# constantingoeldel/alphabeta-rs

Measured on AMD Instinct MI355X. Metric: ABneutral model fits/sec (pedigree x bootstraps x windows), higher is better.
Workload: dtype f64; 1 GPU; C3: synthetic 100-edge/8-generation pedigree (N=105 rows, T=8, K=47 distinct triples), 10 starts + 10000 bootstraps per GPU (bootstraps of one window sharded over the GPUs); rows=105, windows_per_gpu=1, starts=10, bootstraps=10000, plan_device_bytes=9663014, reduction_tree=0x10040, parallelism=bootstraps sharded over 1 GPU(s), one RCCL all-gather of the bootstrap tables

## Files before the change

### alphabeta_rs_amd/csrc/abn_fit_refill.hpp

```cpp
#pragma once
#include "abn_common.hpp"
#include "abn_fit_kernel.hpp"

namespace abn {

constexpr int ST_IDLE = 13;

#ifndef ABN_REFILL_MIN_WAVES
#define ABN_REFILL_MIN_WAVES 3
#endif
template <int G, int RMAX>
__global__ __launch_bounds__(kWave, ABN_REFILL_MIN_WAVES) void abn_fit_refill_kernel(const FitArgs a) {
  static_assert(RMAX > 0, "resident mode only");
  constexpr int NG = kWave / G;
  constexpr int RR = RMAX;
  extern __shared__ __align__(16) double lds[];

  const int lane = threadIdx.x;
  const int g = lane / G;
  const int gl = lane - g * G;
  const int dim = gl & 3;
  const unsigned total = (unsigned)((long long)a.W * a.C);
  const int N = a.N, K = a.K, TP = a.TP;

  double* pw = lds + (size_t)g * a.chain_stride;
  double* dtab = pw + kPw * TP;
  double* wconst = dtab + ((K + 1) & ~1);
  double* dobs = wconst + 4;
  uint32_t* tri_s = reinterpret_cast<uint32_t*>(dobs + ((N + 1) & ~1));

  unsigned* const pht = a.quantum > 0 ? a.park_ht + (blockIdx.x & (kParkShards - 1)) * kParkHeaderInts : nullptr;
  int* const pk = a.quantum > 0 ? a.parked + (size_t)(blockIdx.x & (kParkShards - 1)) * a.park_cap : nullptr;
  const bool canon = a.tree == kTreeCanon;
  uint32_t tidp[(RR + 1) / 2];
  for (int t = gl; t < K; t += G) tri_s[t] = a.tri[t];
#pragma unroll
  for (int q = 0; q < (RR + 1) / 2; ++q) tidp[q] = 0u;
#pragma unroll
  for (int q = 0; q < RR; ++q) {
    const int i = gl + G * q;
    if (i < N) tidp[q / 2] |= (uint32_t)a.tid[i] << (16 * (q & 1));
  }

  unsigned chain = blockIdx.x * NG + g;
  double vx[5], c[5];
  int st = ST_IDLE;
  int iter = 0, evals = 0;
  double xc = 0.0, x0 = 0.0, xr = 0.0, bx = __builtin_nan("");
  double fr = 0.0, best_cost = __builtin_inf();
  bool have_best = false;
  int fin_status = 2;
  int q_start = 0;
  bool fresh_done = false;
  bool wave_fd = false;
  bool tail_mode = false;
  bool tail_park = false;
  unsigned wstep = 0;
#pragma unroll
  for (int k = 0; k < 5; ++k) {
    vx[k] = 0.0;
    c[k] = 0.0;
  }

  auto setup_chain = [&]() {
    const int w = (int)(chain / (unsigned)a.C);
    const int j = (int)(chain - (unsigned)w * (unsigned)a.C);
    const int wi = w * a.wstride;
    const size_t wN = (size_t)w * (size_t)N;
    if (gl == 0) {
      const double p_uu0 = a.p_uu[wi];
      wconst[0] = p_uu0;
      wconst[1] = 1.0 - p_uu0;
      wconst[2] = a.eqp[wi];
      wconst[3] = a.eqp_w[wi] * (double)N;
    }
    const uint32_t* idx_row = (a.dmode == 1) ? a.idx + (size_t)chain * (size_t)N : nullptr;
    const size_t dN = (a.dmode == 2) ? (size_t)chain * (size_t)N : wN;
#pragma unroll
    for (int q = 0; q < RR; ++q) {
      const int i = gl + G * q;
      if (i < N)
        dobs[i] = (a.dmode == 1) ? a.pred[wN + i] + a.resid[wN + idx_row[i]] : a.D[dN + i];
    }
    if (a.smode == 0) {
      const double* s0 = a.simplex0 + (size_t)chain * 20;
#pragma unroll
      for (int k = 0; k < 5; ++k) vx[k] = s0[4 * k + dim];
    } else {
      const uint32_t k0 = (uint32_t)a.seed, k1 = (uint32_t)(a.seed >> 32);
      const uint32_t wg = a.wid ? a.wid[w] : a.window_offset + (uint32_t)w, bg = a.boot_offset + (uint32_t)j;
      vx[0] = a.model[4 * w + dim];
#pragma unroll
      for (int v = 1; v < 5; ++v) {
        uint32_t r[4];
        philox4x32_10((uint32_t)(v - 1) * 2u + (uint32_t)(dim >> 1), bg, wg, kTagJitter, k0, k1, r);
        const uint32_t r0 = r[0], r1 = r[1], r2 = r[2], r3 = r[3];
        const bool odd = (dim & 1) != 0;
        vx[v] = vary_one(vx[0], odd ? r2 : r0, odd ? r3 : r1);
      }
    }
    iter = 0;
    evals = 0;
    bx = __builtin_nan("");
    best_cost = __builtin_inf();
    have_best = false;
    fin_status = 2;
    fr = 0.0;
    q_start = a.quantum > 0 ? -(int)((chain * 2654435761u >> 16) % (unsigned)a.quantum) : 0;
    st = ST_INIT0;
  };
  auto resume_chain = [&]() {
    const int w = (int)(chain / (unsigned)a.C);
    const int wi = w * a.wstride;
    const size_t wN = (size_t)w * (size_t)N;
    if (gl == 0) {
      const double p_uu0 = a.p_uu[wi];
      wconst[0] = p_uu0;
      wconst[1] = 1.0 - p_uu0;
      wconst[2] = a.eqp[wi];
      wconst[3] = a.eqp_w[wi] * (double)N;
    }
    const uint32_t* idx_row = (a.dmode == 1) ? a.idx + (size_t)chain * (size_t)N : nullptr;
    const size_t dN = (a.dmode == 2) ? (size_t)chain * (size_t)N : wN;
#pragma unroll
    for (int q = 0; q < RR; ++q) {
      const int i = gl + G * q;
      if (i < N)
        dobs[i] = (a.dmode == 1) ? a.pred[wN + i] + a.resid[wN + idx_row[i]] : a.D[dN + i];
    }
    double* sp = a.state + (size_t)chain * 32;
    auto ld = [&](int i) { return __hip_atomic_load(sp + i, __ATOMIC_RELAXED, __HIP_MEMORY_SCOPE_AGENT); };
#pragma unroll
    for (int k = 0; k < 5; ++k) {
      vx[k] = ld(4 * k + dim);
      c[k] = ld(20 + k);
    }
    bx = ld(25 + dim);
    best_cost = ld(29);
    const long long ie = __double_as_longlong(ld(30));
    iter = (int)(ie & 0xffffffffll);
    evals = (int)(ie >> 32);
    have_best = __double_as_longlong(ld(31)) != 0;
    fin_status = 2;
    fr = 0.0;
    double acc = vx[0];
    acc = acc + vx[1];
    acc = acc + vx[2];
    acc = acc + vx[3];
    x0 = acc * (1.0 / 4.0);
    xr = x0 + (x0 - vx[4]) * 1.0;
    xc = xr;
    q_start = evals;
    st = ST_REFLECT;
  };
  if (chain < total) setup_chain();
  __syncthreads();

  auto eval = [&](double xd) -> double {
    const double al = dpp_mov<kDppQuadBcast0>(xd), be = dpp_mov<kDppQuadBcast1>(xd);
    const double wt = dpp_mov<kDppQuadBcast2>(xd), ic = dpp_mov<kDppQuadBcast3>(xd);
    const double p_mm = wconst[1];
    const double sv0 = wconst[0], sv1 = wt * p_mm, sv2 = (1.0 - wt) * p_mm;
    const double puu = p_uu_est(al, be);
    const double dq = puu - wconst[2];
    const double pen = wconst[3] * (dq * dq);
    uint32_t tr = tri_s[gl < K ? gl : 0];
    if constexpr (kMatrixFma && G == kWave) build_power_table_mx<G>(al, be, a.T, lds, a.chain_stride, dtab, lane);
    else build_power_table<G>(genmatrix(al, be), a.T, TP, pw, gl);
    __syncthreads();
#pragma unroll 1
    for (int t = gl; t < K; t += G) {
      const uint32_t trn = tri_s[t + G < K ? t + G : 0];
      dtab[t] = triple_dt(tr, pw, TP, sv0, sv1, sv2);
      tr = trn;
    }
    __syncthreads();
    double acc = 0.0;
    constexpr int RC = RR < 8 ? RR : 8;
    constexpr int NA = kWave / G;
    double av[NA];
#pragma unroll
    for (int j = 0; j < NA; ++j) av[j] = 0.0;
#pragma unroll
    for (int q0 = 0; q0 < RR; q0 += RC) {
      double dv[RC], tv[RC], x[RC];
#pragma unroll
      for (int q = 0; q < RC; ++q) {
        const int i = gl + G * (q0 + q);
        dv[q] = dobs[i < N ? i : N - 1];
        tv[q] = dtab[(tidp[(q0 + q) / 2] >> (16 * ((q0 + q) & 1))) & 0xffffu];
      }
#pragma unroll
      for (int q = 0; q < RC; ++q) {
        const double r = dv[q] - ic - tv[q];
        const double term = r * r + pen;
        x[q] = ((gl + G * (q0 + q)) < N) ? term : 0.0;
      }
      if (canon) {
#pragma unroll
        for (int q = 0; q < RC; ++q) av[(q0 + q) % NA] = av[(q0 + q) % NA] + x[q];
      } else {
#pragma unroll
        for (int q = 0; q < RC; ++q) acc = acc + x[q];
      }
    }
    acc = canon ? tree64_finish<G>(av) : group_sum_dpp<G>(acc);
    __syncthreads();
    return acc;
  };

  auto begin_iteration = [&](bool count_iter) {
    const double c_best = c[0];
    if (c_best < best_cost || (__builtin_isinf(c_best) && __builtin_isinf(best_cost) &&
                               (__builtin_signbit(c_best) == __builtin_signbit(best_cost)))) {
      bx = vx[0];
      best_cost = c_best;
      have_best = true;
    }
    if (count_iter) ++iter;
    bool converged = false;
    if (!((c[4] - c[0]) > a.gap_tol)) {
      double sum = 0.0;
#pragma unroll
      for (int k = 0; k < 5; ++k) sum = sum + c[k];
      const double c0 = sum / 5.0;
      double ss = 0.0;
#pragma unroll
      for (int k = 0; k < 5; ++k) ss = ss + (c[k] - c0) * (c[k] - c0);
      const double sd = __builtin_sqrt(1.0 / (5.0 - 1.0) * ss);
      converged = sd < a.sd_tol;
    }
    int status = -1;
    if (converged) status = 0;
    else if (iter >= a.max_iters) status = 1;
    else if (best_cost <= -__builtin_inf()) status = 3;
    bool suspend = false;
    if (a.quantum > 0 && status < 0 && evals - q_start >= a.quantum) {
      int verdict = 0;
      if (gl == 0) {
        const unsigned fq = __hip_atomic_load(a.queue, __ATOMIC_RELAXED, __HIP_MEMORY_SCOPE_AGENT);
        const int av = __hip_atomic_load(reinterpret_cast<int*>(pht) + kParkAvail, __ATOMIC_RELAXED,
                                         __HIP_MEMORY_SCOPE_AGENT);
        const unsigned tl = __hip_atomic_load(pht + kParkTail, __ATOMIC_RELAXED, __HIP_MEMORY_SCOPE_AGENT);
        verdict = ((gridDim.x * NG + fq < total || av > 0) && tl + gridDim.x * NG / kParkShards + NG < a.park_cap) ? 1 : 0;
      }
      suspend = __builtin_amdgcn_ds_bpermute(4 * (g * G), verdict) != 0;
      q_start = evals;
    }
    tail_park = false;
    if (tail_mode && status < 0 && !suspend) {
      suspend = true;
      tail_park = true;
    }
    const bool done = status >= 0 || suspend;
    fin_status = (status >= 0) ? (have_best ? status : 2) : (suspend ? kFitSuspended : fin_status);
    double acc = vx[0];
    acc = acc + vx[1];
    acc = acc + vx[2];
    acc = acc + vx[3];
    x0 = acc * (1.0 / 4.0);
    xr = x0 + (x0 - vx[4]) * 1.0;
    xc = xr;
    st = done ? ST_DONE : ST_REFLECT;
  };

#ifdef ABN_MEASUREMENT_KNOBS
  int prio_cur = 0;
#endif
  while (__ballot(st != ST_IDLE) != 0ull) {
#ifdef ABN_MEASUREMENT_KNOBS
    if (a.prio_mode != 0) {
      const int e = st != ST_IDLE ? evals : 0;
      int m = 0;
#pragma unroll
      for (int j = 0; j < NG; ++j) {
        const int ej = __builtin_amdgcn_readlane(e, j * G);
        m = ej > m ? ej : m;
      }
      int lvl = (m >= a.prio_t[0] ? 1 : 0) + (m >= a.prio_t[1] ? 1 : 0) + (m >= a.prio_t[2] ? 1 : 0);
      if (a.prio_mode == 2) lvl = 3 - lvl;
      if (lvl != prio_cur) {
        prio_cur = lvl;
        if (lvl == 0) __builtin_amdgcn_s_setprio(0);
        else if (lvl == 1) __builtin_amdgcn_s_setprio(1);
        else if (lvl == 2) __builtin_amdgcn_s_setprio(2);
        else __builtin_amdgcn_s_setprio(3);
      }
    }
#endif
    if (a.tail_cap > 0 && wave_fd && !tail_mode && (++wstep & 63u) == 0u) {
      int t = 0;
      if (lane == 0) {
        const unsigned fq = __hip_atomic_load(a.queue, __ATOMIC_RELAXED, __HIP_MEMORY_SCOPE_AGENT);
        const int av = __hip_atomic_load(reinterpret_cast<int*>(pht) + kParkAvail, __ATOMIC_RELAXED, __HIP_MEMORY_SCOPE_AGENT);
        const unsigned fin = __hip_atomic_load(a.slice_status + 1, __ATOMIC_RELAXED, __HIP_MEMORY_SCOPE_AGENT);
        t = (gridDim.x * NG + fq >= total && av <= 0 && total - fin <= (unsigned)a.tail_cap) ? 1 : 0;
      }
      tail_mode = __builtin_amdgcn_readfirstlane(t) != 0;
    }
    const bool in_init = st < ST_REFLECT;
    const double f = eval(in_init ? vx[0] : xc);
    const bool is_ref = st == ST_REFLECT, is_exp = st == ST_EXPAND, is_con = st == ST_CONTRACT;
    const bool active = is_ref || is_exp || is_con;
    const bool acc_r = is_ref && (f < c[3]) && (f >= c[0]);
    const bool go_exp = is_ref && !acc_r && (f < c[0]);
    const bool go_con = is_ref && !acc_r && !go_exp && (f >= c[3]);
    const bool nan_ref = is_ref && !acc_r && !go_exp && !go_con;
    const bool keep_r = is_exp && !(f < fr);
    const bool acc_c = is_con && (f < c[4]);
    const bool rej_c = is_con && !acc_c;
    const bool do_insert = acc_r || is_exp || acc_c;
    const bool start_shrink = nan_ref || (rej_c && a.shrink_variant != 0);
    const bool do_begin = do_insert || (rej_c && a.shrink_variant == 0);
    evals += active ? 1 : 0;
    if (rej_c && a.shrink_variant == 0 && a.no_skip == 0) {
      const int rest = a.max_iters - iter - 1;
      evals += 2 * rest;
      iter += rest;
      if (a.skipped && gl == 0 && rest > 0) atomicAdd(a.skipped, 2ull * (unsigned long long)rest);
    }
    const double xi = keep_r ? xr : xc;
    const double fi = keep_r ? fr : f;
    fr = is_ref ? f : fr;
    const double x_e = x0 + (xr - x0) * 2.0;
    const double x_c = x0 + (vx[4] - x0) * 0.5;
    xc = go_exp ? x_e : (go_con ? x_c : xc);
    st = go_exp ? ST_EXPAND : (go_con ? ST_CONTRACT : st);
    if (do_insert) {
      c[4] = fi;
      vx[4] = xi;
      insert_tail<4>(c, vx);
    }
    if (do_begin) begin_iteration(true);
    if (in_init) {
      const double tv = vx[0];
#pragma unroll
      for (int q = 0; q < 4; ++q) {
        c[q] = c[q + 1];
        vx[q] = vx[q + 1];
      }
      c[4] = f;
      vx[4] = tv;
      st = st + 1;
      if (st == ST_REFLECT) {
        evals = 5;
        sort5(c, vx);
        begin_iteration(false);
      }
    }
    if (__ballot(start_shrink) != 0ull) {
#pragma unroll 1
      for (int k = 1; k < 5; ++k) {
        const double nv = vx[0] + (vx[1] - vx[0]) * 0.5;
        const double fk = eval(start_shrink ? nv : xc);
        if (start_shrink) {
          ++evals;
#pragma unroll
          for (int q = 1; q < 4; ++q) {
            c[q] = c[q + 1];
            vx[q] = vx[q + 1];
          }
          c[4] = fk;
          vx[4] = nv;
        }
      }
      if (start_shrink) {
        sort5(c, vx);
        begin_iteration(true);
      }
    }
    if (__ballot(st == ST_DONE) != 0ull) {
      const bool fin = st == ST_DONE;
      const double b0 = dpp_mov<kDppQuadBcast0>(bx), b1 = dpp_mov<kDppQuadBcast1>(bx);
      unsigned nxt = 0xffffffffu;
      const bool parking = fin && fin_status == kFitSuspended;
      if (parking) {
        double* sp = a.state + (size_t)chain * 32;
        auto sd = [&](int i, double v) { __hip_atomic_store(sp + i, v, __ATOMIC_RELAXED, __HIP_MEMORY_SCOPE_AGENT); };
        if (gl < 4) {
#pragma unroll
          for (int k = 0; k < 5; ++k) sd(4 * k + gl, vx[k]);
          sd(25 + gl, bx);
        }
        if (gl == 0) {
#pragma unroll
          for (int k = 0; k < 5; ++k) sd(20 + k, c[k]);
          sd(29, best_cost);
          sd(30, __longlong_as_double((long long)(unsigned)iter | ((long long)evals << 32)));
          sd(31, __longlong_as_double(have_best ? 1ll : 0ll));
        }
      } else if (fin) {
        if (gl < 4) a.best[(size_t)chain * 4 + gl] = bx;
        if (gl == 0) {
          if (a.slice_status) atomicAdd(a.slice_status + 1, 1u);
          FitInfoDev fo;
          fo.best_cost = best_cost;
          fo.iters = iter;
          fo.evals = evals;
          fo.status = fin_status;
          fo.lanes = a.tree;
          a.info[chain] = fo;
        }
        if (a.raw) {
          double* ro = a.raw + (size_t)chain * 7;
          if (gl < 4) ro[gl] = bx;
          if (gl == 4) ro[4] = est_mm(b0, b1);
          if (gl == 5) ro[5] = est_um(b0, b1);
          if (gl == 6) ro[6] = p_uu_est(b0, b1);
        }
      }
      if (a.quantum > 0) {
        if (__ballot(parking) != 0ull) asm volatile("s_waitcnt vmcnt(0) ; abn: parked state written through" ::: "memory");
        if (parking && tail_park && gl == 0) {
          a.susp_list[atomicAdd(a.susp_count, 1)] = (int)chain;
          atomicAdd(a.slice_status + 2, 1u);
        }
        if (parking && !tail_park && gl == 0) {
          const unsigned pos = atomicAdd(pht + kParkTail, 1u);
#ifdef ABN_MEASUREMENT_KNOBS
          if (!(a.drop_entry != 0 && pos == 0 && (blockIdx.x & (kParkShards - 1)) == 0))
#endif
          __hip_atomic_store(pk + pos, (int)chain, __ATOMIC_RELAXED, __HIP_MEMORY_SCOPE_AGENT);
          atomicAdd(reinterpret_cast<int*>(pht) + kParkAvail, 1);
        }
      }
      bool take_parked = false;
      if (fin && gl == 0) {
        if (!fresh_done) {
          const unsigned f = gridDim.x * NG + atomicAdd(a.queue, 1u);
          if (f < total) nxt = f;
          else fresh_done = true;
        }
        if (nxt == 0xffffffffu && a.quantum > 0) {
          int* avail = reinterpret_cast<int*>(pht) + kParkAvail;
          bool claimed = false;
          for (int tries = 0; tries < 1024 && !claimed; ++tries) {
            if (atomicSub(avail, 1) > 0) {
              claimed = true;
            } else {
              atomicAdd(avail, 1);
              if (__hip_atomic_load(avail, __ATOMIC_RELAXED, __HIP_MEMORY_SCOPE_AGENT) <= 0) break;
              __builtin_amdgcn_s_sleep(1);
            }
          }
          if (claimed) {
            const unsigned h = atomicAdd(pht + kParkHead, 1u);
            int cpk;
            unsigned spins = 0;
            while ((cpk = __hip_atomic_load(pk + h, __ATOMIC_RELAXED, __HIP_MEMORY_SCOPE_AGENT)) < 0 && spins < (1u << 24)) {
              __builtin_amdgcn_s_sleep(1);
              ++spins;
            }
            if (cpk >= 0) {
              nxt = (unsigned)cpk;
              take_parked = true;
            } else if (a.slice_status) {
              atomicOr(a.slice_status, kSliceErrLostEntry);
            }
          }
        }
      }
      nxt = (unsigned)__builtin_amdgcn_ds_bpermute(4 * (g * G), (int)nxt);
      take_parked = __builtin_amdgcn_ds_bpermute(4 * (g * G), (int)take_parked) != 0;
      fresh_done = __builtin_amdgcn_ds_bpermute(4 * (g * G), (int)fresh_done) != 0;
      wave_fd = wave_fd || (__ballot(fresh_done) != 0ull);
      if (fin) {
        st = ST_IDLE;
        if (nxt < total) {
          chain = nxt;
          if (take_parked) resume_chain();
          else setup_chain();
        }
      }
      __syncthreads();
    }
  }
}

}
```

Measured before the change: 3.103 million fits/s.

## Drop per-chain best tracking and split bounds-masked residual loop into fast path

Removes the running best-point registers (bx, best_cost, have_best) and derives them from the sorted simplex's first vertex when a chain finishes, relying on c[0] being monotone non-increasing. The residual loop in eval now checks a scalar, wave-uniform condition per pair of rows and skips the per-row bounds select when the whole block is in range. It also hoists the fixed-point-skip flag out of the loop. The intent is to cut VGPR pressure and per-eval VALU work. It risks changing semantics if a NaN or non-monotone cost path makes the best-ever value differ from c[0], and parked chains no longer restore best state.

```diff
diff --git a/alphabeta_rs_amd/csrc/abn_fit_refill.hpp b/alphabeta_rs_amd/csrc/abn_fit_refill.hpp
--- a/alphabeta_rs_amd/csrc/abn_fit_refill.hpp
+++ b/alphabeta_rs_amd/csrc/abn_fit_refill.hpp
@@ -46,9 +46,8 @@
   double vx[5], c[5];
   int st = ST_IDLE;
   int iter = 0, evals = 0;
-  double xc = 0.0, x0 = 0.0, xr = 0.0, bx = __builtin_nan("");
-  double fr = 0.0, best_cost = __builtin_inf();
-  bool have_best = false;
+  double xc = 0.0, x0 = 0.0, xr = 0.0;
+  double fr = 0.0;
   int fin_status = 2;
   int q_start = 0;
   bool fresh_done = false;
@@ -101,9 +100,6 @@
     }
     iter = 0;
     evals = 0;
-    bx = __builtin_nan("");
-    best_cost = __builtin_inf();
-    have_best = false;
     fin_status = 2;
     fr = 0.0;
     q_start = a.quantum > 0 ? -(int)((chain * 2654435761u >> 16) % (unsigned)a.quantum) : 0;
@@ -135,12 +131,9 @@
       vx[k] = ld(4 * k + dim);
       c[k] = ld(20 + k);
     }
-    bx = ld(25 + dim);
-    best_cost = ld(29);
     const long long ie = __double_as_longlong(ld(30));
     iter = (int)(ie & 0xffffffffll);
     evals = (int)(ie >> 32);
-    have_best = __double_as_longlong(ld(31)) != 0;
     fin_status = 2;
     fr = 0.0;
     double acc = vx[0];
@@ -190,11 +183,27 @@
         dv[q] = dobs[i < N ? i : N - 1];
         tv[q] = dtab[(tidp[(q0 + q) / 2] >> (16 * ((q0 + q) & 1))) & 0xffffu];
       }
-#pragma unroll
-      for (int q = 0; q < RC; ++q) {
-        const double r = dv[q] - ic - tv[q];
-        const double term = r * r + pen;
-        x[q] = ((gl + G * (q0 + q)) < N) ? term : 0.0;
+      constexpr int RB = RC < 2 ? RC : 2;
+      int n_s = N;
+      asm volatile("" : "+s"(n_s));
+#pragma unroll
+      for (int b0 = 0; b0 < RC; b0 += RB) {
+        if (G * (q0 + b0 + RB) <= n_s) {
+#pragma unroll
+          for (int q = b0; q < b0 + RB; ++q) {
+            const double r = dv[q] - ic - tv[q];
+            x[q] = r * r + pen;
+          }
+        } else {
+          int row0 = gl + G * (q0 + b0);
+          asm("" : "+v"(row0));
+#pragma unroll
+          for (int q = b0; q < b0 + RB; ++q) {
+            const double r = dv[q] - ic - tv[q];
+            const double term = r * r + pen;
+            x[q] = (row0 + G * (q - b0) < N) ? term : 0.0;
+          }
+        }
       }
       if (canon) {
 #pragma unroll
@@ -210,13 +219,6 @@
   };
 
   auto begin_iteration = [&](bool count_iter) {
-    const double c_best = c[0];
-    if (c_best < best_cost || (__builtin_isinf(c_best) && __builtin_isinf(best_cost) &&
-                               (__builtin_signbit(c_best) == __builtin_signbit(best_cost)))) {
-      bx = vx[0];
-      best_cost = c_best;
-      have_best = true;
-    }
     if (count_iter) ++iter;
     bool converged = false;
     if (!((c[4] - c[0]) > a.gap_tol)) {
@@ -233,7 +235,7 @@
     int status = -1;
     if (converged) status = 0;
     else if (iter >= a.max_iters) status = 1;
-    else if (best_cost <= -__builtin_inf()) status = 3;
+    else if (c[0] <= -__builtin_inf()) status = 3;
     bool suspend = false;
     if (a.quantum > 0 && status < 0 && evals - q_start >= a.quantum) {
       int verdict = 0;
@@ -253,7 +255,7 @@
       tail_park = true;
     }
     const bool done = status >= 0 || suspend;
-    fin_status = (status >= 0) ? (have_best ? status : 2) : (suspend ? kFitSuspended : fin_status);
+    fin_status = (status >= 0) ? ((c[0] == c[0]) ? status : 2) : (suspend ? kFitSuspended : fin_status);
     double acc = vx[0];
     acc = acc + vx[1];
     acc = acc + vx[2];
@@ -264,6 +266,7 @@
     st = done ? ST_DONE : ST_REFLECT;
   };
 
+  const bool fixed_point_skip = a.shrink_variant == 0 && a.no_skip == 0;
 #ifdef ABN_MEASUREMENT_KNOBS
   int prio_cur = 0;
 #endif
@@ -313,7 +316,7 @@
     const bool start_shrink = nan_ref || (rej_c && a.shrink_variant != 0);
     const bool do_begin = do_insert || (rej_c && a.shrink_variant == 0);
     evals += active ? 1 : 0;
-    if (rej_c && a.shrink_variant == 0 && a.no_skip == 0) {
+    if (rej_c && fixed_point_skip) {
       const int rest = a.max_iters - iter - 1;
       evals += 2 * rest;
       iter += rest;
@@ -371,6 +374,9 @@
     }
     if (__ballot(st == ST_DONE) != 0ull) {
       const bool fin = st == ST_DONE;
+      const bool have_best = c[0] == c[0];
+      const double bx = have_best ? vx[0] : __builtin_nan("");
+      const double best_cost = have_best ? c[0] : __builtin_inf();
       const double b0 = dpp_mov<kDppQuadBcast0>(bx), b1 = dpp_mov<kDppQuadBcast1>(bx);
       unsigned nxt = 0xffffffffu;
       const bool parking = fin && fin_status == kFitSuspended;
```

Result: no change. 3.121 million fits/s (median of 3 runs) (+0.6%).
